# flucoma/flucoma-core

Hardware: AMD Instinct MI355X
Metric: NMF iterations/sec (buffer-iterations over the whole BufNMF job: STFT + 200-iter KL-NMF + write-back), rank-32 fft2048 (higher is better)
Workload: dtype f64; 1 GPU; BASELINE config 4 shard: 128 x 10 s mono 44.1 kHz buffers per GPU, fft 2048 / hop 512, rank 32, 200 iterations, seed 42; buffers_per_gpu=128, samples=441000, frames=862, bins=1025, rank=32, parallelism=single

## Files before the change

### flucoma-core_amd/csrc/kernels_nmf5.hip

```cpp
#include "fluhip_kernels.h"
#include "recip_tree.h"

#include <cstdlib>

namespace fluhip {

typedef double d2 __attribute__((ext_vector_type(2)));

struct Upd5Args
{
  const double* V;
  int64_t ldv, strideV;
  const double* Mv;
  int64_t strideM;
  double* S;
  int64_t strideS;
  int R, C, B;
  int nGroups, wavesPerBuf, wgPerBuf, nSteps, nsplit, stepsPerSplit;
  double* part;
  double* dpart;
  int64_t Cp;
  int xcdMap;
  const double* nrm;
  int nrmMode;
  double* statPart;
  long long* clk;
  const WaveDesc* list;
  double* sidePart;
  double* sideWold;
  const double* cmbStat;
  const double* cmbSide;
  const double* cmbWold;
  double* cmbNrmOut;
  double* cmbRowOut;
  int cmbParts, cmbSlices, cmbK;
  const double* colIn;
  double* colOut;
  int colInN;
};

#ifndef FLUHIP_QUOTIENT_CORRECTION
#define FLUHIP_QUOTIENT_CORRECTION 0
#endif
constexpr bool kQuotientCorrection = FLUHIP_QUOTIENT_CORRECTION != 0;
#ifndef FLUHIP_SHARED_RECIPROCAL
#define FLUHIP_SHARED_RECIPROCAL 1
#endif
constexpr bool kSharedReciprocal = FLUHIP_SHARED_RECIPROCAL != 0;
#ifndef FLUHIP_RCP_GROUP
#define FLUHIP_RCP_GROUP 4
#endif
constexpr int kRcpGroup = FLUHIP_RCP_GROUP;
#ifndef FLUHIP_QV_M10
#define FLUHIP_QV_M10 1
#endif
static_assert(kRcpGroup == 2 || kRcpGroup == 4 || kRcpGroup == 8, "quotients per reciprocal");
#ifndef FLUHIP_EPILOGUE_SC1
#define FLUHIP_EPILOGUE_SC1 1
#endif
__device__ __forceinline__ void store_result16(double* p, double __attribute__((ext_vector_type(2))) t)
{
#if FLUHIP_EPILOGUE_SC1 == 2
  asm volatile("global_store_dwordx4 %0, %1, off sc1 nt\n\ts_nop 1" ::"v"(p), "v"(t) : "memory");
#elif FLUHIP_EPILOGUE_SC1 == 3
  asm volatile("global_store_dwordx4 %0, %1, off nt\n\ts_nop 1" ::"v"(p), "v"(t) : "memory");
#elif FLUHIP_EPILOGUE_SC1 == 4
  asm volatile("global_store_dwordx4 %0, %1, off sc0 sc1\n\ts_nop 1" ::"v"(p), "v"(t) : "memory");
#elif FLUHIP_EPILOGUE_SC1
  asm volatile("global_store_dwordx4 %0, %1, off sc1\n\ts_nop 1" ::"v"(p), "v"(t) : "memory");
#else
  *reinterpret_cast<double __attribute__((ext_vector_type(2)))*>(p) = t;
#endif
}

__device__ __forceinline__ double fdiv_pos(double v, double d)
{
  double y = __builtin_amdgcn_rcp(d);
  const double e = __builtin_fma(-d, y, 1.0);
  y = __builtin_fma(y, e, y);
  const double r = v * y;
  const double res = __builtin_fma(-d, r, v);
  return __builtin_fma(res, y, r);
}

#define FLUHIP_GLDS(src, dst)                                                                     \
  __builtin_amdgcn_global_load_lds((const __attribute__((address_space(1))) void*) (src),          \
                                   (__attribute__((address_space(3))) void*) (dst), 16, 0, 0)

__device__ __forceinline__ void glds16(const void* sbase, unsigned voff, unsigned ldsAddr)
{
  asm volatile("s_mov_b32 m0, %0\n\ts_nop 0\n\tglobal_load_lds_dwordx4 %1, %2"
               :
               : "s"(ldsAddr), "v"(voff), "s"(sbase)
               : "memory", "m0");
}
#ifndef FLUHIP_PARTIAL_STAGED
#define FLUHIP_PARTIAL_STAGED 1
#endif
#ifndef FLUHIP_V_NT
#define FLUHIP_V_NT 1
#endif
__device__ __forceinline__ void glds16_v(const void* sbase, unsigned voff, unsigned ldsAddr)
{
#if FLUHIP_V_NT
  asm volatile("s_mov_b32 m0, %0\n\ts_nop 0\n\tglobal_load_lds_dwordx4 %1, %2 nt"
               :
               : "s"(ldsAddr), "v"(voff), "s"(sbase)
               : "memory", "m0");
#else
  glds16(sbase, voff, ldsAddr);
#endif
}
__device__ __forceinline__ unsigned lds_addr(const void* p)
{
  return (unsigned) (size_t) (__attribute__((address_space(3))) const void*) p;
}

template <int N>
__device__ __forceinline__ void load_vec5(double (&dst)[N], const double* p)
{
#pragma unroll
  for (int j = 0; j < N; j += 2)
  {
    d2 t = *reinterpret_cast<const d2*>(p + j);
    dst[j] = t[0];
    dst[j + 1] = t[1];
  }
}
#ifndef FLUHIP_STATIONARY_NT
#define FLUHIP_STATIONARY_NT 0
#endif
template <int N>
__device__ __forceinline__ void load_stationary5(double (&dst)[N], const double* p)
{
#if FLUHIP_STATIONARY_NT
#pragma unroll
  for (int j = 0; j < N; j += 2)
  {
    d2 t = __builtin_nontemporal_load(reinterpret_cast<const d2*>(p + j));
    dst[j] = t[0];
    dst[j + 1] = t[1];
  }
#else
  load_vec5<N>(dst, p);
#endif
}

template <int CTRL>
__device__ __forceinline__ double quad_dpp(double v)
{
  const long long b = __double_as_longlong(v);
  const int lo = __builtin_amdgcn_update_dpp(0, (int) (b & 0xffffffff), CTRL, 0xf, 0xf, false);
  const int hi = __builtin_amdgcn_update_dpp(0, (int) (b >> 32), CTRL, 0xf, 0xf, false);
  return __longlong_as_double(((long long) hi << 32) | (unsigned) lo);
}

template <int M, int NG, int NS, int WPS, int INSTR = 0, int MODE = 0, int DS = 1, int LIST = 0, int SIDEQ = 0, int KPM = 4 * M>
__global__ __launch_bounds__(256 * WPS, WPS) void nmf_update5_kernel(Upd5Args a)
{
  constexpr int KP = 4 * M;
  static_assert(KPM >= KP && KPM % 16 == 0, "array rank");
  constexpr int SPR = KP / 2;
  constexpr int NJV = (32 * NG + 63) / 64;
  constexpr int NJM = (4 * SPR + 63) / 64;
  constexpr int VSTAGE = NJV * 1024;
  constexpr int MSTAGE = NJM * 1024;
  constexpr int WAVE_LDS = NS * (VSTAGE + MSTAGE);
  constexpr int IPS = NJV + NJM;
  constexpr bool QV = MODE == 1 && (DS == 2 || (DS == 1 && INSTR == 0 && (M == 4 || (M == 6 && NG <= 8) || (M == 8 && NG <= 6) || (FLUHIP_QV_M10 && M == 10 && NG <= 4))));
  constexpr int STG_BYTES = (NG * M + M) * 512;
  constexpr int WAVE_REGION = (LIST != 0 && STG_BYTES > WAVE_LDS && 4 * STG_BYTES <= 160 * 1024) ? STG_BYTES : WAVE_LDS;

  extern __shared__ __attribute__((aligned(16))) char lds[];

  int id = blockIdx.x;
  int buf, wg, split;
  [[maybe_unused]] const WaveDesc* wd = nullptr;
  if constexpr (LIST != 0)
  {
    wd = a.list + ((int64_t) id * 4 * WPS + __builtin_amdgcn_readfirstlane(threadIdx.x >> 6));
    buf = __builtin_amdgcn_readfirstlane(wd->buf);
    wg = 0; split = 0;
  }
  else
  {
  if (a.xcdMap)
  {
    const int xcd = id & 7;
    int slot = id >> 3;
    split = slot % a.nsplit;
    slot /= a.nsplit;
    wg = slot % a.wgPerBuf;
    buf = xcd + 8 * (slot / a.wgPerBuf);
  }
  else
  {
    split = id % a.nsplit;
    wg = (id / a.nsplit) % a.wgPerBuf;
    buf = id / (a.nsplit * a.wgPerBuf);
  }
  if (buf >= a.B) return;
  }
  long long tEntry = 0;
  if constexpr (INSTR) tEntry = (long long) __builtin_amdgcn_s_memrealtime();
  long long clkC0 = 0, clkR0 = 0;
  const bool stamp = a.clk != nullptr && blockIdx.x == 0;
  if (stamp)
  {
    clkC0 = (long long) __builtin_readcyclecounter();
    clkR0 = (long long) __builtin_amdgcn_s_memrealtime();
  }
  const int lane = threadIdx.x & 63;
  const int wave = __builtin_amdgcn_readfirstlane(threadIdx.x >> 6);
  constexpr int WPB = 4 * WPS;
  const int strip = wg * WPB + wave;
  int g0 = 0, ng = 0;
  if constexpr (LIST != 0)
  {
    g0 = __builtin_amdgcn_readfirstlane(wd->g0);
    ng = __builtin_amdgcn_readfirstlane(wd->ng);
  }
  else
  {
  if (strip >= a.wavesPerBuf) return;
  const int base = a.nGroups / a.wavesPerBuf, rem = a.nGroups % a.wavesPerBuf;
  {
    const int nPairs = (a.wavesPerBuf + WPS - 1) / WPS;
    int acc0 = 0;
    for (int st = 0; st <= strip; st++)
    {
      const int wgi = st / WPB, w = st % WPB;
      const int pair = wgi * 4 + (w & 3), member = w >> 2;
      const int extra = (pair + nPairs * member) < rem ? 1 : 0;
      const int cnt = base + extra;
      if (st == strip) { g0 = acc0; ng = cnt; }
      acc0 += cnt;
    }
  }
  }
  if (ng <= 0) return;

  const int x = lane & 3, blk = (lane >> 2) & 3, y = lane >> 4;
  const double* __restrict__ V = a.V + (int64_t) buf * a.strideV;
  const double* __restrict__ Mv = a.Mv + (int64_t) buf * a.strideM;
  double* S = a.S + (int64_t) buf * a.strideS;

  char* vring = lds + wave * WAVE_REGION;
  char* mring = vring + NS * VSTAGE;

  unsigned voffs[NJV];
#pragma unroll
  for (int j = 0; j < NJV; j++)
  {
    int i = 64 * j + lane;
    int row = i / (8 * NG), cc = i % (8 * NG);
    if (row > 3) { row = 3; }
    cc = min(cc, 8 * ng - 1);
    voffs[j] = (unsigned) ((row * a.ldv + cc * 2) * 8);
  }
  unsigned moffs[NJM];
#pragma unroll
  for (int j = 0; j < NJM; j++)
  {
    int p = 64 * j + lane;
    int row = p / SPR, pos = p % SPR;
    if (row > 3) row = 3;
    const int cs = (pos - row + SPR) % SPR;
    const int cx = cs ^ (((cs >> 4) & 3) << 2);
    const int c = cx < SPR ? cx : cs;
    moffs[j] = (unsigned) ((row * KPM + c * 2) * 8);
  }

  int s0, s1;
  if constexpr (LIST != 0)
  {
    s0 = __builtin_amdgcn_readfirstlane(wd->s0);
    s1 = __builtin_amdgcn_readfirstlane(wd->s1);
  }
  else
  {
    s0 = split * a.stepsPerSplit;
    s1 = min(s0 + a.stepsPerSplit, a.nSteps);
  }
  const int sLast = s1 - 1;

  auto issue_stage = [&](int st) {
    const int sc = min(st, sLast);
    const int slot = st % NS;
    const char* vsrc = reinterpret_cast<const char*>(V + (int64_t) sc * 4 * a.ldv + (int64_t) g0 * 16);
    const char* msrc = reinterpret_cast<const char*>(Mv + (int64_t) sc * 4 * KPM);
#pragma unroll
    for (int j = 0; j < NJV; j++) FLUHIP_GLDS(vsrc + voffs[j], vring + slot * VSTAGE + j * 1024);
#pragma unroll
    for (int j = 0; j < NJM; j++) FLUHIP_GLDS(msrc + moffs[j], mring + slot * MSTAGE + j * 1024);
  };

  auto fill_slots = [&](int t0, int t1) {
    if (s0 < s1)
    {
#pragma unroll
      for (int t = t0; t < t1; t++)
      {
        const int sc = min(s0 + t, sLast);
        const char* vsrc = reinterpret_cast<const char*>(V + (int64_t) sc * 4 * a.ldv + (int64_t) g0 * 16);
        const char* msrc = reinterpret_cast<const char*>(Mv + (int64_t) sc * 4 * KPM);
#pragma unroll
        for (int j = 0; j < NJV; j++) FLUHIP_GLDS(vsrc + voffs[j], vring + t * VSTAGE + j * 1024);
#pragma unroll
        for (int j = 0; j < NJM; j++) FLUHIP_GLDS(msrc + moffs[j], mring + t * MSTAGE + j * 1024);
      }
    }
  };
  long long tP1 = 0, tP2 = 0, tP3 = 0;
  if constexpr (INSTR) tP1 = (long long) __builtin_amdgcn_s_memrealtime();
  constexpr int NJSV = SIDEQ ? (NG * 128 + 1023) / 1024 : 0;
  constexpr bool NORMQ = (SIDEQ & 2) != 0;
  [[maybe_unused]] char* sideL = nullptr;
  [[maybe_unused]] double cs[8], cm[8], cn[8], cd[8], cwo = 0.0, cc[8];
  static_assert(DS != 2 || NORMQ || SIDEQ == 0, "DS == 2: the W update's plain form or the H update's norm form");
  if constexpr (DS == 2)
  {
#pragma unroll
    for (int u = 0; u < 8; u++) cc[u] = 0.0;
    if (lane < KP)
    {
      const int64_t rec = NORMQ ? KPM : 2 * KPM;
      const double* cp = a.colIn + (int64_t) buf * a.colInN * rec + (NORMQ ? 0 : KPM) + lane;
#pragma unroll
      for (int u = 0; u < 8; u++) if (u < a.colInN) cc[u] = cp[(int64_t) u * rec];
    }
  }
  if constexpr (NORMQ)
  {
#pragma unroll
    for (int u = 0; u < 8; u++) { cs[u] = 0.0; cm[u] = -INFINITY; cn[u] = 0.0; cd[u] = 0.0; }
    if (lane < KP)
    {
      const double* sp = a.cmbStat + (int64_t) buf * a.cmbParts * 2 * KPM + lane;
      const double* qp = a.cmbSide + (int64_t) buf * a.cmbSlices * 2 * KPM + lane;
      cwo = a.cmbWold[(int64_t) buf * KPM + lane];
#pragma unroll
      for (int u = 0; u < 8; u++)
      {
        if (u < a.cmbParts) { cs[u] = sp[(int64_t) u * 2 * KPM]; cm[u] = sp[(int64_t) u * 2 * KPM + KPM]; }
        if (u < a.cmbSlices) { cn[u] = qp[(int64_t) u * 2 * KPM]; cd[u] = qp[(int64_t) u * 2 * KPM + KPM]; }
      }
    }
  }
  constexpr int SIDE_BYTES = SIDEQ ? (1 + NJSV) * 1024 : 0;
  constexpr int EXTRA_BYTES = SIDE_BYTES + (DS == 2 ? 512 : 0);
  [[maybe_unused]] double* colL = reinterpret_cast<double*>(lds + WPB * WAVE_REGION + wave * EXTRA_BYTES + SIDE_BYTES);
  if constexpr (SIDEQ)
  {
    sideL = lds + WPB * WAVE_REGION + wave * EXTRA_BYTES;
    if constexpr (!NORMQ)
    {
      const char* wsrc = reinterpret_cast<const char*>(Mv + (int64_t) (a.R - 1) * KPM) + min(lane, SPR - 1) * 16;
      FLUHIP_GLDS(wsrc, sideL);
    }
#pragma unroll
    for (int j = 0; j < NJSV; j++)
    {
      const int i = min(64 * j + lane, 8 * ng - 1);
      const char* vsrc = reinterpret_cast<const char*>(V + (int64_t) (a.R - 1) * a.ldv + (int64_t) g0 * 16) + i * 16;
      FLUHIP_GLDS(vsrc, sideL + 1024 + j * 1024);
    }
  }
  if constexpr (MODE >= 1) fill_slots(0, 2);

  double sb[NG][M];
  double acc[NG][M];
#pragma unroll
  for (int g = 0; g < NG; g++)
  {
#pragma unroll
    for (int m = 0; m < M; m++) { acc[g][m] = 0.0; sb[g][m] = 0.0; }
    if (g < ng) load_stationary5<M>(sb[g], S + (int64_t) ((g0 + g) * 16 + 4 * blk + x) * KPM + M * y);
  }
  [[maybe_unused]] double colSum = 0.0;
  if constexpr (DS == 2)
  {
#pragma unroll
    for (int u = 0; u < 8; u++) colSum += cc[u];
    if (lane < KP)
    {
      const int64_t rec = NORMQ ? KPM : 2 * KPM;
      const double* cp = a.colIn + (int64_t) buf * a.colInN * rec + (NORMQ ? 0 : KPM) + lane;
      for (int j = 8; j < a.colInN; j++) colSum += cp[(int64_t) j * rec];
    }
    if constexpr (!NORMQ)
    {
      if (lane < KP) colL[lane] = colSum;
      asm volatile("s_waitcnt lgkmcnt(0)" ::: "memory");
    }
  }
  if constexpr (NORMQ)
  {
    double t = 0.0, mv = -INFINITY, n = 0.0, d = 0.0;
#pragma unroll
    for (int u = 0; u < 8; u++) { t += cs[u]; mv = fmax(mv, cm[u]); n += cn[u]; d += cd[u]; }
    if (lane < KP)
    {
      const double* sp = a.cmbStat + (int64_t) buf * a.cmbParts * 2 * KPM + lane;
      const double* qp = a.cmbSide + (int64_t) buf * a.cmbSlices * 2 * KPM + lane;
      for (int j = 8; j < a.cmbParts; j++) { t += sp[(int64_t) j * 2 * KPM]; mv = fmax(mv, sp[(int64_t) j * 2 * KPM + KPM]); }
      for (int j = 8; j < a.cmbSlices; j++) { n += qp[(int64_t) j * 2 * KPM]; d += qp[(int64_t) j * 2 * KPM + KPM]; }
    }
    const bool liveK = lane < a.cmbK;
    const double wnew = liveK ? (cwo * n) / fmax(d, kEpsilon) : 0.0;
    t = __builtin_fma(wnew, wnew, t);
    mv = liveK ? fmax(mv, wnew) : -INFINITY;
#pragma unroll
    for (int off = 1; off < 64; off <<= 1) mv = fmax(mv, __shfl_xor(mv, off));
    const double nv = (liveK && mv > kEpsilon) ? sqrt(t) : 1.0;
    double* ldsW = reinterpret_cast<double*>(sideL);
    if (lane < KP)
    {
      ldsW[lane] = wnew;
      ldsW[64 + lane] = nv;
      if constexpr (DS == 2) colL[lane] = colSum + wnew;
      a.cmbRowOut[(int64_t) buf * a.strideM + (int64_t) (a.R - 1) * KPM + lane] = wnew;
      if (strip == 0) a.cmbNrmOut[(int64_t) buf * KPM + lane] = nv;
    }
    asm volatile("s_waitcnt lgkmcnt(0)" ::: "memory");
  }
  if (a.nrmMode)
  {
    double nr[M];
    if constexpr (NORMQ)
    {
      const double* ldsN = reinterpret_cast<const double*>(sideL) + 64;
#pragma unroll
      for (int m = 0; m < M; m++) nr[m] = ldsN[M * y + m];
    }
    else
    load_vec5<M>(nr, a.nrm + (int64_t) buf * KPM + M * y);
#pragma unroll
    for (int g = 0; g < NG; g++)
#pragma unroll
      for (int m = 0; m < M; m++) sb[g][m] = fdiv_pos(sb[g][m], nr[m]);
  }
  if constexpr (INSTR)
  {
    __builtin_amdgcn_sched_barrier(0);
    asm volatile("" ::"v"(sb[0][0]), "v"(sb[NG - 1][M - 1]));
    tP2 = (long long) __builtin_amdgcn_s_memrealtime();
    __builtin_amdgcn_sched_barrier(0);
  }
  if constexpr (MODE >= 1) fill_slots(2, NS);
  double dsum[M];
#pragma unroll
  for (int m = 0; m < M; m++) dsum[m] = 0.0;

  auto slot_of = [](int c, int r) { const int cx = c ^ (((c >> 4) & 3) << 2); return ((cx < SPR ? cx : c) + r) % SPR; };
  int maOff[M / 2], mbOff[M / 2];
#pragma unroll
  for (int j = 0; j < M / 2; j++)
  {
    maOff[j] = x * (KP * 8) + slot_of((M / 2) * y + j, x) * 16;
    mbOff[j] = y * (KP * 8) + slot_of((M / 2) * x + j, y) * 16;
  }
  const int vOff = y * (NG * 128) + (4 * blk + x) * 8;

  auto read_ma = [&](int st, double (&ma)[M]) {
    const char* mp = mring + (st % NS) * MSTAGE;
#pragma unroll
    for (int j = 0; j < M / 2; j++)
    {
      d2 t = *reinterpret_cast<const d2*>(mp + maOff[j]);
      ma[2 * j] = t[0];
      ma[2 * j + 1] = t[1];
    }
  };
  auto read_v = [&](int st, double (&v)[NG]) {
    const char* vp = vring + (st % NS) * VSTAGE + vOff;
#pragma unroll
    for (int g = 0; g < NG; g++) v[g] = *reinterpret_cast<const double*>(vp + g * 128);
  };
  auto read_mb = [&](int st, double (&mb)[M]) {
    const char* mp = mring + (st % NS) * MSTAGE;
#pragma unroll
    for (int j = 0; j < M / 2; j++)
    {
      d2 t = *reinterpret_cast<const d2*>(mp + mbOff[j]);
      mb[2 * j] = t[0];
      mb[2 * j + 1] = t[1];
    }
  };

  constexpr int P0 = (NG >= 5) ? 1 : (NG >= 3 ? 2 : (NG >= 2 ? 4 : 8));
  constexpr int P = (M % P0 == 0 || M < P0) ? P0 : (M == 12 ? P0 / 2 : P0);
  auto q_phase = [&](const double (&ma)[M], double (&q)[NG]) {
    constexpr int PP = (P <= M) ? P : M;
    double qp[NG][PP];
#pragma unroll
    for (int g = 0; g < NG; g++)
#pragma unroll
      for (int p = 0; p < PP; p++) qp[g][p] = 0.0;
#pragma unroll
    for (int m = 0; m < M; m++)
#pragma unroll
      for (int g = 0; g < NG; g++)
        qp[g][m % PP] = __builtin_amdgcn_mfma_f64_4x4x4f64(ma[m], sb[g][m], qp[g][m % PP], 0, 0, 0);
#pragma unroll
    for (int g = 0; g < NG; g++)
    {
      double t = qp[g][0];
#pragma unroll
      for (int p = 1; p < PP; p++) t += qp[g][p];
      q[g] = t;
    }
  };
  auto ratio_phase = [&](const double (&v)[NG], const double (&q)[NG], double (&ratio)[NG]) {
    double d[NG], yv[NG];
#pragma unroll
    for (int g = 0; g < NG; g++) d[g] = q[g] > kEpsilon ? q[g] : kEpsilon;
    if constexpr (kQuotientCorrection || !kSharedReciprocal)
    {
#pragma unroll
      for (int g = 0; g < NG; g++) yv[g] = __builtin_amdgcn_rcp(d[g]);
#pragma unroll
      for (int g = 0; g < NG; g++) ratio[g] = __builtin_fma(-d[g], yv[g], 1.0);
#pragma unroll
      for (int g = 0; g < NG; g++) yv[g] = __builtin_fma(yv[g], ratio[g], yv[g]);
    }
    else if constexpr (kRcpGroup > 2)
    {
      recip_tree<NG, kRcpGroup>(d, yv);
    }
    else
    {
      constexpr int NP = NG / 2;
      double pr[NP > 0 ? NP : 1], rr[NP > 0 ? NP : 1], ee[NP > 0 ? NP : 1];
#pragma unroll
      for (int h = 0; h < NP; h++) pr[h] = d[2 * h] * d[2 * h + 1];
#pragma unroll
      for (int h = 0; h < NP; h++) rr[h] = __builtin_amdgcn_rcp(pr[h]);
      if constexpr (NG & 1) yv[NG - 1] = __builtin_amdgcn_rcp(d[NG - 1]);
#pragma unroll
      for (int h = 0; h < NP; h++) ee[h] = __builtin_fma(-pr[h], rr[h], 1.0);
      if constexpr (NG & 1) ratio[NG - 1] = __builtin_fma(-d[NG - 1], yv[NG - 1], 1.0);
#pragma unroll
      for (int h = 0; h < NP; h++) rr[h] = __builtin_fma(rr[h], ee[h], rr[h]);
      if constexpr (NG & 1) yv[NG - 1] = __builtin_fma(yv[NG - 1], ratio[NG - 1], yv[NG - 1]);
#pragma unroll
      for (int h = 0; h < NP; h++)
      {
        yv[2 * h] = rr[h] * d[2 * h + 1];
        yv[2 * h + 1] = rr[h] * d[2 * h];
      }
    }
#pragma unroll
    for (int g = 0; g < NG; g++) ratio[g] = v[g] * yv[g];
    if constexpr (kQuotientCorrection)
    {
#pragma unroll
      for (int g = 0; g < NG; g++) d[g] = __builtin_fma(-d[g], ratio[g], v[g]);
#pragma unroll
      for (int g = 0; g < NG; g++) ratio[g] = __builtin_fma(d[g], yv[g], ratio[g]);
    }
  };
  auto out_phase = [&](const double (&ratio)[NG], const double (&mb)[M]) {
#pragma unroll
    for (int g = 0; g < NG; g++)
#pragma unroll
      for (int m = 0; m < M; m++) acc[g][m] = __builtin_amdgcn_mfma_f64_4x4x4f64(ratio[g], mb[m], acc[g][m], 0, 0, 0);
#pragma unroll
    for (int m = 0; m < M; m++) if constexpr (DS == 1) dsum[m] += mb[m];
  };

  if constexpr (MODE == 2)
  {
    if (s0 < s1)
    {
      static_assert(NS >= 4, "overlapped pipeline: ring depth >= 4");
      const unsigned vringA = __builtin_amdgcn_readfirstlane(lds_addr(vring));
      const unsigned mringA = __builtin_amdgcn_readfirstlane(lds_addr(mring));
      const char* vAddr = vring + vOff;
      const char* maAddr[M / 2];
      const char* mbAddr[M / 2];
#pragma unroll
      for (int j = 0; j < M / 2; j++) { maAddr[j] = mring + maOff[j]; mbAddr[j] = mring + mbOff[j]; }
      double v[NG], ma[M], mb[M], qA[NG], qB[NG];
      asm volatile("s_waitcnt vmcnt(%0)" ::"n"((NS - 2) * IPS) : "memory");
#pragma unroll
      for (int j = 0; j < M / 2; j++)
      {
        d2 t = *reinterpret_cast<const d2*>(maAddr[j]);
        ma[2 * j] = t[0]; ma[2 * j + 1] = t[1];
      }
      q_phase(ma, qA);
#pragma unroll
      for (int g = 0; g < NG; g++) v[g] = *reinterpret_cast<const double*>(vAddr + g * 128);
#pragma unroll
      for (int j = 0; j < M / 2; j++)
      {
        d2 t = *reinterpret_cast<const d2*>(mbAddr[j]);
        mb[2 * j] = t[0]; mb[2 * j + 1] = t[1];
        d2 t2 = *reinterpret_cast<const d2*>(maAddr[j] + MSTAGE);
        ma[2 * j] = t2[0]; ma[2 * j + 1] = t2[1];
      }
      constexpr int NMF = M * NG;
// ... 252 lines not shown
#pragma unroll
            for (int p = 1; p < PP; p++) t += qp[g][p];
            qn[g] = t;
          }
        }
        const long long c4 = tick();
        if constexpr (INSTR) { tWait += c1 - c0; tRatio += c2 - c1; tQ += c3 - c2; tOut += c4 - c3; }
      };
      for (int s = s0; s < s1; s += NS)
      {
#pragma unroll
        for (int u = 0; u < NS; u++)
        {
          if (s + u >= s1) break;
          if (u % 2 == 0) half(s + u, u, (u + 1) % NS, (u + 2) % NS, vX, maX, mbX, vY, maY, mbY, qA, qB);
          else half(s + u, u, (u + 1) % NS, (u + 2) % NS, vY, maY, mbY, vX, maX, mbX, qB, qA);
        }
      }
      asm volatile("s_waitcnt vmcnt(0)" ::: "memory");
      if constexpr (INSTR)
      {
        const long long tLoop1 = (long long) __builtin_amdgcn_s_memrealtime();
        tReal += tLoop1;
        if (blockIdx.x == 17 && threadIdx.x == 0 && a.dpart)
        {
          long long* o = reinterpret_cast<long long*>(a.dpart);
          o[0] = tWait; o[1] = 0; o[2] = tRatio; o[3] = tQ; o[4] = tOut; o[5] = 0; o[6] = s1 - s0; o[7] = tReal;
        }
        if (threadIdx.x == 0 && a.dpart && (blockIdx.x & 63) == 17)
        {
          long long* o = reinterpret_cast<long long*>(a.dpart) + 16 + 4 * (blockIdx.x >> 6);
          o[0] = tEntry; o[1] = tLoop0; o[2] = tLoop1;
          if (blockIdx.x == 17) { long long* q = reinterpret_cast<long long*>(a.dpart) + 12; q[0] = tP1; q[1] = tP2; q[2] = tP3; }
        }
      }
    }
  }
  else
  if (s0 < s1)
  {
#pragma unroll
    for (int t = 0; t < NS; t++) issue_stage(s0 + t);
    double ma[M], mb[M], v[NG], qA[NG], qB[NG], ratio[NG];
    asm volatile("s_waitcnt vmcnt(%0)" ::"n"((NS - 1) * IPS) : "memory");
    read_ma(s0, ma);
    q_phase(ma, qA);
    long long tWait = 0, tRead = 0, tRatio = 0, tQ = 0, tOut = 0, tDma = 0;
    auto tick = [&]() -> long long {
      if constexpr (INSTR) { __builtin_amdgcn_sched_barrier(0); long long c = __builtin_readcyclecounter(); __builtin_amdgcn_sched_barrier(0); return c; }
      return 0;
    };
    for (int s = s0; s < s1; s += 2)
    {
      long long c0 = tick();
      asm volatile("s_waitcnt vmcnt(%0)" ::"n"((NS - 2) * IPS) : "memory");
      long long c1 = tick();
      read_v(s, v);
      read_ma(s + 1, ma);
      read_mb(s, mb);
      asm volatile("s_waitcnt lgkmcnt(0)" ::: "memory");
      long long c2 = tick();
      issue_stage(s + NS);
      long long c3 = tick();
      ratio_phase(v, qA, ratio);
      long long c4 = tick();
      q_phase(ma, qB);
      long long c5 = tick();
      out_phase(ratio, mb);
      long long c6 = tick();
      if constexpr (INSTR) { tWait += c1 - c0; tRead += c2 - c1; tDma += c3 - c2; tRatio += c4 - c3; tQ += c5 - c4; tOut += c6 - c5; }
      if (s + 1 < s1)
      {
        asm volatile("s_waitcnt vmcnt(%0)" ::"n"((NS - 2) * IPS) : "memory");
        read_v(s + 1, v);
        read_ma(s + 2, ma);
        read_mb(s + 1, mb);
        asm volatile("s_waitcnt lgkmcnt(0)" ::: "memory");
        issue_stage(s + 1 + NS);
        ratio_phase(v, qB, ratio);
        q_phase(ma, qA);
        out_phase(ratio, mb);
      }
    }
    asm volatile("s_waitcnt vmcnt(0)" ::: "memory");
    if constexpr (INSTR)
    {
      if (blockIdx.x == 17 && threadIdx.x == 0 && a.dpart)
      {
        long long* o = reinterpret_cast<long long*>(a.dpart);
        o[0] = tWait; o[1] = tRead; o[2] = tRatio; o[3] = tQ; o[4] = tOut; o[5] = tDma; o[6] = (s1 - s0 + 1) / 2;
      }
    }
  }

  [[maybe_unused]] int lPart = -1, lStat = 0, lD = -1;
  if constexpr (LIST != 0 && 4 * STG_BYTES <= 160 * 1024)
  {
    const int grp = __builtin_amdgcn_readfirstlane(wd->grp);
    if (grp >> 16)
    {
      const int leader = grp & 15, rank = (grp >> 4) & 15, gsize = (grp >> 8) & 15;
      double* mine = reinterpret_cast<double*>(lds + wave * WAVE_REGION);
      if (rank > 0)
      {
#pragma unroll
        for (int g = 0; g < NG; g++)
#pragma unroll
          for (int m = 0; m < M; m++) mine[(g * M + m) * 64 + lane] = acc[g][m];
#pragma unroll
        for (int m = 0; m < M; m++) mine[(NG * M + m) * 64 + lane] = dsum[m];
      }
      __syncthreads();
      if (rank > 0) return;
      for (int r = 1; r < gsize; r++)
      {
        const double* src = reinterpret_cast<const double*>(lds + (leader + r) * WAVE_REGION);
#pragma unroll
        for (int g = 0; g < NG; g++)
#pragma unroll
          for (int m = 0; m < M; m++) acc[g][m] += src[(g * M + m) * 64 + lane];
#pragma unroll
        for (int m = 0; m < M; m++) dsum[m] += src[(NG * M + m) * 64 + lane];
      }
    }
  }
  if constexpr (LIST != 0)
  {
    lPart = __builtin_amdgcn_readfirstlane(wd->partIdx);
    lStat = __builtin_amdgcn_readfirstlane(wd->statIdx);
    lD = __builtin_amdgcn_readfirstlane(wd->dIdx);
  }
  auto whole = [&]() -> bool { if constexpr (LIST != 0) return lPart < 0; else return a.nsplit == 1; };
  if constexpr (DS == 1)
  {
#pragma unroll
    for (int m = 0; m < M; m++)
    {
      double d = dsum[m];
      d += __shfl_xor(d, 16);
      d += __shfl_xor(d, 32);
      dsum[m] = d;
    }
  }
  else if constexpr (DS == 2)
  {
#pragma unroll
    for (int m = 0; m < M; m++) dsum[m] = colL[M * x + m];
  }
  else if (whole())
  {
    load_vec5<M>(dsum, a.dpart + (int64_t) buf * KPM + M * x);
  }

  if (whole())
  {
    double nrE[M], ss[M], mx[M];
    [[maybe_unused]] double csum[M];
    constexpr bool COLOUT = DS == 2 && !NORMQ;
    [[maybe_unused]] double nrL = 1.0;
    if constexpr (NORMQ)
    {
      const double* ldsN = reinterpret_cast<const double*>(sideL) + 64;
#pragma unroll
      for (int m = 0; m < M; m++) nrE[m] = ldsN[M * x + m];
      if (lane < KP) nrL = ldsN[lane];
    }
    else
    {
      if (a.nrmMode) load_vec5<M>(nrE, a.nrm + (int64_t) buf * KPM + M * x);
      if constexpr (SIDEQ) if (strip == 0 && lane < KP) nrL = a.nrm[(int64_t) buf * KPM + lane];
    }
    if (a.nrmMode == 2)
    {
#pragma unroll
      for (int m = 0; m < M; m++) dsum[m] = fdiv_pos(dsum[m], nrE[m]);
    }
    double dd[M], dy[M];
#pragma unroll
    for (int m = 0; m < M; m++)
    {
      dd[m] = fmax(dsum[m], kEpsilon);
      double y0 = __builtin_amdgcn_rcp(dd[m]);
      dy[m] = __builtin_fma(y0, __builtin_fma(-dd[m], y0, 1.0), y0);
      ss[m] = 0.0;
      mx[m] = -INFINITY;
      if constexpr (COLOUT) csum[m] = 0.0;
    }
    const int srcLane = y + 4 * blk + 16 * x;
    constexpr int ROWB = KP * 8 + 16;
    constexpr int GRPB = 16 * ROWB;
    constexpr int GB = (WAVE_LDS / GRPB) >= NG ? NG : (WAVE_LDS / GRPB);
    static_assert(GB >= 1, "result staging does not fit the ring");
    constexpr int CPR = KP / 2;
    constexpr int NST = 16 * CPR / 64;
    char* stg = lds + wave * WAVE_REGION;
    [[maybe_unused]] double wsd[M], numS[M], denS[M], vsd[NG];
    if constexpr (SIDEQ)
    {
      static_assert(KP <= 64 && LIST == 0, "side-column partials: one lane per component at the end");
      const double* wl = reinterpret_cast<const double*>(sideL);
      const double* vl = reinterpret_cast<const double*>(sideL + 1024);
#pragma unroll
      for (int m = 0; m < M; m++) { wsd[m] = fdiv_pos(wl[M * x + m], nrE[m]); numS[m] = 0.0; denS[m] = 0.0; }
#pragma unroll
      for (int g = 0; g < NG; g++)
      {
        const int col = (g0 + g) * 16 + 4 * blk + y;
        vsd[g] = (g < ng && col < a.C) ? vl[g * 16 + 4 * blk + y] : 0.0;
      }
    }
#pragma unroll
    for (int gb = 0; gb < NG; gb += GB)
    {
#pragma unroll
      for (int g = gb; g < gb + GB && g < NG; g++)
      {
        const int col = (g0 + g) * 16 + 4 * blk + y;
        const bool live = g < ng && col < a.C;
        char* row = stg + (g - gb) * GRPB + (4 * blk + y) * ROWB + (M * x) * 8;
        [[maybe_unused]] double rr[M];
#pragma unroll
        for (int m = 0; m < M; m += 2)
        {
          double r2[2];
#pragma unroll
          for (int e = 0; e < 2; e++)
          {
            const double so = __shfl(sb[g][m + e], srcLane);
            const double v = so * acc[g][m + e];
            const double r0 = v * dy[m + e];
            const double r = __builtin_fma(__builtin_fma(-dd[m + e], r0, v), dy[m + e], r0);
            r2[e] = r;
            if constexpr (SIDEQ) rr[m + e] = r;
            if (live)
            {
              ss[m + e] = __builtin_fma(r, r, ss[m + e]);
              mx[m + e] = fmax(mx[m + e], r);
              if constexpr (COLOUT) csum[m + e] += r;
            }
          }
          *reinterpret_cast<d2*>(row + m * 8) = d2{r2[0], r2[1]};
        }
        if constexpr (SIDEQ)
        {
          double qs = 0.0;
#pragma unroll
          for (int m = 0; m < M; m++) qs = __builtin_fma(rr[m], wsd[m], qs);
          qs += quad_dpp<0xB1>(qs);
          qs += quad_dpp<0x4E>(qs);
          const double ratio = live ? fdiv_pos(vsd[g], fmax(qs, kEpsilon)) : 0.0;
#pragma unroll
          for (int m = 0; m < M; m++)
          {
            numS[m] = __builtin_fma(ratio, rr[m], numS[m]);
            denS[m] += live ? rr[m] : 0.0;
          }
        }
      }
#pragma unroll
      for (int g = gb; g < gb + GB && g < NG; g++)
      {
        if (g < ng)
        {
#pragma unroll
          for (int j = 0; j < NST; j++)
          {
            const int c = 64 * j + lane;
            const int r = c / CPR, piece = c % CPR;
            const d2 t = *reinterpret_cast<const d2*>(stg + (g - gb) * GRPB + r * ROWB + piece * 16);
            const int col = (g0 + g) * 16 + r;
            if (col < a.C) store_result16(S + (int64_t) col * KPM + piece * 2, t);
          }
        }
      }
    }
    if constexpr (SIDEQ)
    {
      double* red = reinterpret_cast<double*>(stg);
      asm volatile("s_waitcnt lgkmcnt(0)" ::: "memory");
      const int jr = 4 * blk + y;
#pragma unroll
      for (int m = 0; m < M; m++)
      {
        red[jr * KP + M * x + m] = numS[m];
        red[(16 + jr) * KP + M * x + m] = denS[m];
      }
      asm volatile("s_waitcnt lgkmcnt(0)" ::: "memory");
      if (lane < KP)
      {
        double pn[16], pd[16];
#pragma unroll
        for (int j = 0; j < 16; j++) { pn[j] = red[j * KP + lane]; pd[j] = red[(16 + j) * KP + lane]; }
        double n = 0.0, d = 0.0;
#pragma unroll
        for (int j = 0; j < 16; j++) { n += pn[j]; d += pd[j]; }
        double* sp = a.sidePart + ((int64_t) buf * a.wavesPerBuf + strip) * 2 * KPM;
        sp[lane] = n;
        sp[KPM + lane] = d;
        if (strip == 0) a.sideWold[(int64_t) buf * KPM + lane] = reinterpret_cast<const double*>(sideL)[lane] / nrL;
      }
    }
    if (a.statPart)
    {
#pragma unroll
      for (int m = 0; m < M; m++)
      {
        double t = ss[m], u = mx[m];
#pragma unroll
        for (int off = 4; off < 64; off <<= 1)
        {
          t += __shfl_xor(t, off);
          u = fmax(u, __shfl_xor(u, off));
        }
        ss[m] = t;
        mx[m] = u;
      }
      if (lane < 4)
      {
        double* sp = a.statPart + (LIST ? (int64_t) lStat : ((int64_t) buf * a.wavesPerBuf + strip)) * 2 * KPM + M * x;
#pragma unroll
        for (int m = 0; m < M; m++) { sp[m] = ss[m]; sp[KPM + m] = mx[m]; }
      }
    }
    if constexpr (COLOUT)
    {
#pragma unroll
      for (int m = 0; m < M; m++)
      {
        double t = csum[m];
#pragma unroll
        for (int off = 4; off < 64; off <<= 1) t += __shfl_xor(t, off);
        csum[m] = t;
      }
      if (lane < 4)
      {
        double* cp = a.colOut + ((int64_t) buf * a.wavesPerBuf + strip) * KPM + M * x;
#pragma unroll
        for (int m = 0; m < M; m++) cp[m] = csum[m];
      }
    }
  }
  else
  {
    double* part = a.part + (LIST ? (int64_t) lPart : ((int64_t) buf * a.nsplit + split)) * a.Cp * KPM;
#if FLUHIP_PARTIAL_STAGED
    {
      constexpr int ROWB = KP * 8 + 16;
      constexpr int GRPB = 16 * ROWB;
      constexpr int GB = (WAVE_LDS / GRPB) >= NG ? NG : (WAVE_LDS / GRPB);
      static_assert(GB >= 1, "partial staging does not fit the ring");
      constexpr int CPR = KP / 2, NST = 16 * CPR / 64;
      char* stg = lds + wave * WAVE_REGION;
#pragma unroll
      for (int gb = 0; gb < NG; gb += GB)
      {
#pragma unroll
        for (int g = gb; g < gb + GB && g < NG; g++)
        {
          char* row = stg + (g - gb) * GRPB + (4 * blk + y) * ROWB + (M * x) * 8;
#pragma unroll
          for (int m = 0; m < M; m += 2) *reinterpret_cast<d2*>(row + m * 8) = d2{acc[g][m], acc[g][m + 1]};
        }
#pragma unroll
        for (int g = gb; g < gb + GB && g < NG; g++)
        {
          if (g < ng)
          {
#pragma unroll
            for (int j = 0; j < NST; j++)
            {
              const int c = 64 * j + lane;
              const int r = c / CPR, piece = c % CPR;
              const d2 t = *reinterpret_cast<const d2*>(stg + (g - gb) * GRPB + r * ROWB + piece * 16);
              store_result16(part + (int64_t) ((g0 + g) * 16 + r) * KPM + piece * 2, t);
            }
          }
        }
      }
    }
#else
#pragma unroll
    for (int g = 0; g < NG; g++)
    {
      if (g < ng)
      {
        const int col = (g0 + g) * 16 + 4 * blk + y;
        double* pp = part + (int64_t) col * KPM + M * x;
#pragma unroll
        for (int m = 0; m < M; m++) pp[m] = acc[g][m];
      }
    }
#endif
    if (DS && (LIST ? lD >= 0 : strip == 0) && blk == 0 && y == 0)
    {
      double* dp = a.dpart + (LIST ? (int64_t) lD : ((int64_t) buf * a.nsplit + split)) * KPM + M * x;
#pragma unroll
      for (int m = 0; m < M; m++) dp[m] = dsum[m];
    }
  }
  if (stamp && threadIdx.x == 0)
  {
    __builtin_amdgcn_s_waitcnt(0);
    const long long c1 = (long long) __builtin_readcyclecounter(), r1 = (long long) __builtin_amdgcn_s_memrealtime();
    a.clk[0] += 1;
    a.clk[1] += c1 - clkC0;
    a.clk[2] += r1 - clkR0;
  }
  if constexpr (INSTR)
  {
    __builtin_amdgcn_s_waitcnt(0);
    if (threadIdx.x == 0 && a.dpart && (blockIdx.x & 63) == 17)
      reinterpret_cast<long long*>(a.dpart)[16 + 4 * (blockIdx.x >> 6) + 3] = (long long) __builtin_amdgcn_s_memrealtime();
  }
}


template <int M, int NG, int NS, int MODE, int KPM = 4 * M>
static void launch5_list(const UpdateArgs& a, hipStream_t s)
{
  Upd5Args k{};
  k.V = a.V; k.ldv = a.ldv; k.strideV = a.strideV;
  k.Mv = a.Mv; k.strideM = a.strideM;
  k.S = a.S; k.strideS = a.strideS;
  k.R = a.R; k.C = a.C; k.B = a.B;
  k.nGroups = (a.C + 15) / 16;
  k.wavesPerBuf = 1; k.wgPerBuf = 1; k.nSteps = (a.R + 3) / 4; k.nsplit = 1; k.stepsPerSplit = k.nSteps;
  k.part = a.part; k.dpart = a.dpart; k.Cp = a.Cp;
  k.nrm = a.nrm; k.nrmMode = a.nrmMode; k.statPart = a.listPartial ? nullptr : a.statPart;
  k.clk = a.clk; k.xcdMap = 0; k.list = a.list;
  constexpr int KP = 4 * M, SPR = KP / 2;
  constexpr int NJV = (32 * NG + 63) / 64, NJM = (4 * SPR + 63) / 64;
  constexpr size_t ring = (size_t) NS * (NJV + NJM) * 1024, stg = (size_t) (NG * M + M) * 512;
  constexpr size_t shmem = 4 * ((stg > ring && 4 * stg <= 160 * 1024) ? stg : ring);
  static_assert(shmem <= 160 * 1024, "LDS");
  auto kern = nmf_update5_kernel<M, NG, NS, 1, 0, MODE, 1, 1, 0, KPM>;
  request_dynamic_lds(kern, (size_t) (shmem));
  hipLaunchKernelGGL(kern, dim3((unsigned) a.listWGs), dim3(256), shmem, s, k);
}

template <int M, int NG, int NS, int WPS, int INSTR = 0, int MODE = 0, int DS = 1, int SIDEQ = 0, int KPM = 4 * M>
static void launch5_t(const UpdateArgs& a, int wavesPerBuf, hipStream_t s)
{
  Upd5Args k;
  if (a.dryRun) return;
  k.sidePart = SIDEQ ? a.sideOut : nullptr; k.sideWold = SIDEQ ? a.sideWold : nullptr;
  k.cmbStat = a.cmbStat; k.cmbSide = a.cmbSide; k.cmbWold = a.cmbWold; k.cmbNrmOut = a.cmbNrmOut; k.cmbRowOut = a.cmbRowOut;
  k.cmbParts = a.cmbParts; k.cmbSlices = a.cmbSlices; k.cmbK = a.cmbK;
  k.colIn = a.colIn; k.colOut = a.colOut; k.colInN = a.colInN;
  k.V = a.V; k.ldv = a.ldv; k.strideV = a.strideV;
  k.Mv = a.Mv; k.strideM = a.strideM;
  k.S = a.S; k.strideS = a.strideS;
  k.R = a.R; k.C = a.C; k.B = a.B;
  k.nGroups = (a.C + 15) / 16;
  k.wavesPerBuf = wavesPerBuf;
  k.wgPerBuf = (wavesPerBuf + 4 * WPS - 1) / (4 * WPS);
  k.nSteps = (a.R + 3) / 4;
  k.nsplit = a.nsplit < 1 ? 1 : a.nsplit;
  k.stepsPerSplit = (k.nSteps + k.nsplit - 1) / k.nsplit;
  k.part = a.part; k.dpart = a.dpart; k.Cp = a.Cp;
  k.nrm = a.nrm; k.nrmMode = a.nrmMode; k.statPart = a.nsplit > 1 ? nullptr : a.statPart;
  k.clk = a.clk;
  k.xcdMap = a.B >= 8 ? 1 : 0;
  k.list = nullptr;
  const int bufs = k.xcdMap ? (int) round_up(a.B, 8) : a.B;
  const unsigned grid = (unsigned) (bufs * k.wgPerBuf * k.nsplit);
  constexpr int KP = 4 * M, SPR = KP / 2;
  constexpr int NJV = (32 * NG + 63) / 64, NJM = (4 * SPR + 63) / 64;
  constexpr size_t shmem = (size_t) 4 * WPS * ((NS * (NJV + NJM) + (SIDEQ ? 1 + (NG * 128 + 1023) / 1024 : 0)) * 1024 + (DS == 2 ? 512 : 0));
  static_assert(shmem <= 160 * 1024, "LDS ring does not fit");
  auto kern = nmf_update5_kernel<M, NG, NS, WPS, INSTR, MODE, DS, 0, SIDEQ, KPM>;
  request_dynamic_lds(kern, (size_t) (shmem));
  hipLaunchKernelGGL(kern, dim3(grid), dim3(256 * WPS), shmem, s, k);
  if (k.nsplit > 1)
    launch_update_finalize(a.S, a.strideS, a.part, a.dpart, a.C, a.Kp, a.Cp, k.nsplit, a.B, s, a.nrm, a.nrmMode,
                           a.statPart);
}

#ifndef FLUHIP_K5_OFFSIZE_TU
static int max_groups(int M)
{
  if (M <= 8) return 9;
  if (M <= 16) return 4;
  return 2;
}

int nmf_update5_waves_per_buffer(int C, int Kp, int B)
{
  const int M = Kp / 4, G = (C + 15) / 16, ngmax = max_groups(M);
  const int wmin = (G + ngmax - 1) / ngmax;
  static const int forceW = [] { const char* e = fluhip::ab_getenv("FLUHIP_PLAN_W"); return e ? std::atoi(e) : 0; }();
  if (forceW > 0) return forceW < wmin ? wmin : (forceW > G ? G : forceW);
  int w = wmin;
  const int simds = 1024;
  if ((int64_t) B * w >= simds)
  {
    for (int cand = wmin; cand <= wmin + 2 && cand <= G; cand++)
      if (((int64_t) B * cand) % simds == 0) { w = cand; break; }
  }
  else
  {
    const int64_t wfill = (simds + B - 1) / B;
    if (wfill <= G / 3 || wfill <= wmin)
      w = (int) std::max<int64_t>(wmin, wfill);
    else
      w = std::max(wmin, (G + 2) / 3);
    if (w > G) w = G;
    if (w < 1) w = 1;
  }
  return w;
}


#endif

template <int M, int NG, int WPS>
constexpr int ring_depth()
{
  constexpr int NJ = (32 * NG + 63) / 64 + (4 * (2 * M) + 63) / 64;
  constexpr int fit = 160 / (4 * WPS * NJ);
  return fit >= 6 ? 6 : (fit < 3 ? 3 : fit);
}

#ifndef FLUHIP_K5_OFFSIZE_TU
template <int M, int NG, int WPS>
static int launch5_ng(const UpdateArgs& a, int w, int ng, hipStream_t s)
{
  if constexpr (NG == 1) launch5_t<M, 1, ring_depth<M, 1, WPS>(), WPS>(a, w, s);
  else
  {
    const bool sideq = a.sideOut && a.sideWold && a.nrmMode == 2 && a.nsplit <= 1 && w <= kSideFromHSlots;
// ... 254 lines not shown
```

Baseline: 244,900 iterations/s.

## Software-pipeline epilogue staging with double-buffered LDS areas and scalar-base immediate-offset stores

Restructures the update kernel's epilogue so each 16-column group's results are staged into one of two LDS areas while the previous group is read back and stored to global memory, replacing the batch-then-store loop. Global stores now use an SGPR base plus a 32-bit lane offset and compile-time immediate offsets, which cuts 64-bit address arithmetic per store. The side-quotient math can be deferred behind the stores, and shuffle batching is tuned by M. An optional flag (off by default) moves the ring prefill earlier. Risks are higher register pressure and changed LDS reuse hazards when only one staging area fits.

```diff
diff --git a/flucoma-core_amd/csrc/kernels_nmf5.hip b/flucoma-core_amd/csrc/kernels_nmf5.hip
--- a/flucoma-core_amd/csrc/kernels_nmf5.hip
+++ b/flucoma-core_amd/csrc/kernels_nmf5.hip
@@ -2,6 +2,7 @@
 #include "recip_tree.h"
 
 #include <cstdlib>
+#include <type_traits>
 
 namespace fluhip {
 
@@ -58,19 +59,33 @@
 #ifndef FLUHIP_EPILOGUE_SC1
 #define FLUHIP_EPILOGUE_SC1 1
 #endif
-__device__ __forceinline__ void store_result16(double* p, double __attribute__((ext_vector_type(2))) t)
-{
 #if FLUHIP_EPILOGUE_SC1 == 2
-  asm volatile("global_store_dwordx4 %0, %1, off sc1 nt\n\ts_nop 1" ::"v"(p), "v"(t) : "memory");
+#define FLUHIP_STORE_POLICY " sc1 nt"
 #elif FLUHIP_EPILOGUE_SC1 == 3
-  asm volatile("global_store_dwordx4 %0, %1, off nt\n\ts_nop 1" ::"v"(p), "v"(t) : "memory");
+#define FLUHIP_STORE_POLICY " nt"
 #elif FLUHIP_EPILOGUE_SC1 == 4
-  asm volatile("global_store_dwordx4 %0, %1, off sc0 sc1\n\ts_nop 1" ::"v"(p), "v"(t) : "memory");
-#elif FLUHIP_EPILOGUE_SC1
-  asm volatile("global_store_dwordx4 %0, %1, off sc1\n\ts_nop 1" ::"v"(p), "v"(t) : "memory");
+#define FLUHIP_STORE_POLICY " sc0 sc1"
 #else
-  *reinterpret_cast<double __attribute__((ext_vector_type(2)))*>(p) = t;
-#endif
+#define FLUHIP_STORE_POLICY " sc1"
+#endif
+template <int IMM>
+__device__ __forceinline__ void store_result16(const char* sbase, unsigned voff, double __attribute__((ext_vector_type(2))) t)
+{
+  static_assert(IMM >= 0 && IMM < 4096, "immediate offset of a global store");
+#if FLUHIP_EPILOGUE_SC1
+  asm volatile("global_store_dwordx4 %0, %1, %2 offset:%3" FLUHIP_STORE_POLICY "\n\ts_nop 1" ::"v"(voff), "v"(t), "s"(sbase), "n"(IMM) : "memory");
+#else
+  *reinterpret_cast<double __attribute__((ext_vector_type(2)))*>(const_cast<char*>(sbase) + voff + IMM) = t;
+#endif
+}
+template <int J, int N, class F>
+__device__ __forceinline__ void static_for5(F&& f)
+{
+  if constexpr (J < N)
+  {
+    f(std::integral_constant<int, J>{});
+    static_for5<J + 1, N>(f);
+  }
 }
 
 __device__ __forceinline__ double fdiv_pos(double v, double d)
@@ -129,6 +144,9 @@
 }
 #ifndef FLUHIP_STATIONARY_NT
 #define FLUHIP_STATIONARY_NT 0
+#endif
+#ifndef FLUHIP_EARLY_RING
+#define FLUHIP_EARLY_RING 0
 #endif
 template <int N>
 __device__ __forceinline__ void load_stationary5(double (&dst)[N], const double* p)
@@ -377,6 +395,12 @@
     for (int m = 0; m < M; m++) { acc[g][m] = 0.0; sb[g][m] = 0.0; }
     if (g < ng) load_stationary5<M>(sb[g], S + (int64_t) ((g0 + g) * 16 + 4 * blk + x) * KPM + M * y);
   }
+  [[maybe_unused]] double nrFirst[M];
+  if constexpr (MODE >= 1 && FLUHIP_EARLY_RING)
+  {
+    if constexpr (!NORMQ) if (a.nrmMode) load_vec5<M>(nrFirst, a.nrm + (int64_t) buf * KPM + M * y);
+    fill_slots(2, NS);
+  }
   [[maybe_unused]] double colSum = 0.0;
   if constexpr (DS == 2)
   {
@@ -433,6 +457,11 @@
 #pragma unroll
       for (int m = 0; m < M; m++) nr[m] = ldsN[M * y + m];
     }
+    else if constexpr (MODE >= 1 && FLUHIP_EARLY_RING)
+    {
+#pragma unroll
+      for (int m = 0; m < M; m++) nr[m] = nrFirst[m];
+    }
     else
     load_vec5<M>(nr, a.nrm + (int64_t) buf * KPM + M * y);
 #pragma unroll
@@ -447,7 +476,7 @@
     tP2 = (long long) __builtin_amdgcn_s_memrealtime();
     __builtin_amdgcn_sched_barrier(0);
   }
-  if constexpr (MODE >= 1) fill_slots(2, NS);
+  if constexpr (MODE >= 1 && !FLUHIP_EARLY_RING) fill_slots(2, NS);
   double dsum[M];
 #pragma unroll
   for (int m = 0; m < M; m++) dsum[m] = 0.0;
@@ -1006,6 +1035,44 @@
     load_vec5<M>(dsum, a.dpart + (int64_t) buf * KPM + M * x);
   }
 
+  constexpr int ROWB = KP * 8 + 16;
+  constexpr int GRPB = 16 * ROWB;
+  static_assert(WAVE_LDS >= GRPB, "result staging does not fit the ring");
+  constexpr int NAREA = WAVE_LDS >= 2 * GRPB ? 2 : 1;
+  constexpr int CPR = KP / 2;
+  constexpr int NST = 16 * CPR / 64;
+  constexpr int NSB = M <= 8 ? NST : (M <= 14 ? 4 : 1);
+  char* const stg = lds + wave * WAVE_REGION;
+  auto read_pieces = [&](const char* area, auto jb, d2 (&t)[NSB]) __attribute__((always_inline)) {
+    constexpr int j0 = decltype(jb)::value * NSB, jn = (NST - j0) < NSB ? (NST - j0) : NSB;
+#pragma unroll
+    for (int j = 0; j < jn; j++)
+    {
+      const int c = 64 * (j0 + j) + lane, r = c / CPR, piece = c % CPR;
+      t[j] = *reinterpret_cast<const d2*>(area + r * ROWB + piece * 16);
+    }
+  };
+  auto store_pieces = [&](const double* dst, int rowsLive, auto jb, const d2 (&t)[NSB]) __attribute__((always_inline)) {
+    constexpr int j0 = decltype(jb)::value * NSB, jn = (NST - j0) < NSB ? (NST - j0) : NSB;
+    const char* db = reinterpret_cast<const char*>(dst);
+    auto put = [&](auto jc, bool guard) __attribute__((always_inline)) {
+      constexpr int j = j0 + decltype(jc)::value;
+      const int c = 64 * j + lane, r = c / CPR, piece = c % CPR;
+      if (guard && r >= rowsLive) return;
+      if constexpr (KPM == KP) store_result16<(j & 3) * 1024>(db + (j >> 2) * 4096, (unsigned) lane * 16u, t[j - j0]);
+      else store_result16<0>(db, (unsigned) ((r * KPM + piece * 2) * 8), t[j - j0]);
+    };
+    if (rowsLive >= 16) static_for5<0, jn>([&](auto jc) { put(jc, false); });
+    else static_for5<0, jn>([&](auto jc) { put(jc, true); });
+  };
+  auto store_group = [&](const char* area, const double* dst, int rowsLive) __attribute__((always_inline)) {
+    static_for5<0, (NST + NSB - 1) / NSB>([&](auto jb) {
+      d2 t[NSB];
+      read_pieces(area, jb, t);
+      store_pieces(dst, rowsLive, jb, t);
+    });
+  };
+
   if (whole())
   {
     double nrE[M], ss[M], mx[M];
@@ -1041,13 +1108,6 @@
       if constexpr (COLOUT) csum[m] = 0.0;
     }
     const int srcLane = y + 4 * blk + 16 * x;
-    constexpr int ROWB = KP * 8 + 16;
-    constexpr int GRPB = 16 * ROWB;
-    constexpr int GB = (WAVE_LDS / GRPB) >= NG ? NG : (WAVE_LDS / GRPB);
-    static_assert(GB >= 1, "result staging does not fit the ring");
-    constexpr int CPR = KP / 2;
-    constexpr int NST = 16 * CPR / 64;
-    char* stg = lds + wave * WAVE_REGION;
     [[maybe_unused]] double wsd[M], numS[M], denS[M], vsd[NG];
     if constexpr (SIDEQ)
     {
@@ -1063,69 +1123,69 @@
         vsd[g] = (g < ng && col < a.C) ? vl[g * 16 + 4 * blk + y] : 0.0;
       }
     }
-#pragma unroll
-    for (int gb = 0; gb < NG; gb += GB)
-    {
-#pragma unroll
-      for (int g = gb; g < gb + GB && g < NG; g++)
-      {
-        const int col = (g0 + g) * 16 + 4 * blk + y;
-        const bool live = g < ng && col < a.C;
-        char* row = stg + (g - gb) * GRPB + (4 * blk + y) * ROWB + (M * x) * 8;
-        [[maybe_unused]] double rr[M];
-#pragma unroll
-        for (int m = 0; m < M; m += 2)
+    [[maybe_unused]] double rr[M];
+    constexpr int SHB = M <= 8 ? M : 2;
+    constexpr bool SIDE_LATE = M <= 14;
+    auto side_math = [&](int g) __attribute__((always_inline)) {
+      const int col = (g0 + g) * 16 + 4 * blk + y;
+      const bool live = col < a.C;
+      double qs = 0.0;
+#pragma unroll
+      for (int m = 0; m < M; m++) qs = __builtin_fma(rr[m], wsd[m], qs);
+      qs += quad_dpp<0xB1>(qs);
+      qs += quad_dpp<0x4E>(qs);
+      const double ratio = live ? fdiv_pos(vsd[g], fmax(qs, kEpsilon)) : 0.0;
+#pragma unroll
+      for (int m = 0; m < M; m++)
+      {
+        numS[m] = __builtin_fma(ratio, rr[m], numS[m]);
+        denS[m] += live ? rr[m] : 0.0;
+      }
+    };
+    auto group_math = [&](int g) __attribute__((always_inline)) {
+      const int col = (g0 + g) * 16 + 4 * blk + y;
+      const bool live = col < a.C;
+      char* row = stg + (g % NAREA) * GRPB + (4 * blk + y) * ROWB + (M * x) * 8;
+      double so[SHB];
+#pragma unroll
+      for (int m = 0; m < M; m += 2)
+      {
+        if (m % SHB == 0)
         {
-          double r2[2];
-#pragma unroll
-          for (int e = 0; e < 2; e++)
+#pragma unroll
+          for (int u = 0; u < SHB; u++) so[u] = __shfl(sb[g][m + u], srcLane);
+        }
+        double r2[2];
+#pragma unroll
+        for (int e = 0; e < 2; e++)
+        {
+          const double v = so[(m + e) % SHB] * acc[g][m + e];
+          const double r0 = v * dy[m + e];
+          const double r = __builtin_fma(__builtin_fma(-dd[m + e], r0, v), dy[m + e], r0);
+          r2[e] = r;
+          if constexpr (SIDEQ) rr[m + e] = r;
+          if (live)
           {
-            const double so = __shfl(sb[g][m + e], srcLane);
-            const double v = so * acc[g][m + e];
-            const double r0 = v * dy[m + e];
-            const double r = __builtin_fma(__builtin_fma(-dd[m + e], r0, v), dy[m + e], r0);
-            r2[e] = r;
-            if constexpr (SIDEQ) rr[m + e] = r;
-            if (live)
-            {
-              ss[m + e] = __builtin_fma(r, r, ss[m + e]);
-              mx[m + e] = fmax(mx[m + e], r);
-              if constexpr (COLOUT) csum[m + e] += r;
-            }
-          }
-          *reinterpret_cast<d2*>(row + m * 8) = d2{r2[0], r2[1]};
-        }
-        if constexpr (SIDEQ)
-        {
-          double qs = 0.0;
-#pragma unroll
-          for (int m = 0; m < M; m++) qs = __builtin_fma(rr[m], wsd[m], qs);
-          qs += quad_dpp<0xB1>(qs);
-          qs += quad_dpp<0x4E>(qs);
-          const double ratio = live ? fdiv_pos(vsd[g], fmax(qs, kEpsilon)) : 0.0;
-#pragma unroll
-          for (int m = 0; m < M; m++)
-          {
-            numS[m] = __builtin_fma(ratio, rr[m], numS[m]);
-            denS[m] += live ? rr[m] : 0.0;
+            ss[m + e] = __builtin_fma(r, r, ss[m + e]);
+            mx[m + e] = fmax(mx[m + e], r);
+            if constexpr (COLOUT) csum[m + e] += r;
           }
         }
-      }
-#pragma unroll
-      for (int g = gb; g < gb + GB && g < NG; g++)
-      {
-        if (g < ng)
-        {
-#pragma unroll
-          for (int j = 0; j < NST; j++)
-          {
-            const int c = 64 * j + lane;
-            const int r = c / CPR, piece = c % CPR;
-            const d2 t = *reinterpret_cast<const d2*>(stg + (g - gb) * GRPB + r * ROWB + piece * 16);
-            const int col = (g0 + g) * 16 + r;
-            if (col < a.C) store_result16(S + (int64_t) col * KPM + piece * 2, t);
-          }
-        }
+        *reinterpret_cast<d2*>(row + m * 8) = d2{r2[0], r2[1]};
+      }
+    };
+#pragma unroll
+    for (int g = 0; g <= NG; g++)
+    {
+      if (g > 0 && g - 1 < ng)
+      {
+        store_group(stg + ((g - 1) % NAREA) * GRPB, S + (int64_t) (g0 + g - 1) * 16 * KPM, a.C - (g0 + g - 1) * 16);
+        if constexpr (SIDEQ && SIDE_LATE) side_math(g - 1);
+      }
+      if (g < NG && g < ng)
+      {
+        group_math(g);
+        if constexpr (SIDEQ && !SIDE_LATE) side_math(g);
       }
     }
     if constexpr (SIDEQ)
@@ -1198,38 +1258,15 @@
   {
     double* part = a.part + (LIST ? (int64_t) lPart : ((int64_t) buf * a.nsplit + split)) * a.Cp * KPM;
 #if FLUHIP_PARTIAL_STAGED
-    {
-      constexpr int ROWB = KP * 8 + 16;
-      constexpr int GRPB = 16 * ROWB;
-      constexpr int GB = (WAVE_LDS / GRPB) >= NG ? NG : (WAVE_LDS / GRPB);
-      static_assert(GB >= 1, "partial staging does not fit the ring");
-      constexpr int CPR = KP / 2, NST = 16 * CPR / 64;
-      char* stg = lds + wave * WAVE_REGION;
-#pragma unroll
-      for (int gb = 0; gb < NG; gb += GB)
-      {
-#pragma unroll
-        for (int g = gb; g < gb + GB && g < NG; g++)
-        {
-          char* row = stg + (g - gb) * GRPB + (4 * blk + y) * ROWB + (M * x) * 8;
-#pragma unroll
-          for (int m = 0; m < M; m += 2) *reinterpret_cast<d2*>(row + m * 8) = d2{acc[g][m], acc[g][m + 1]};
-        }
-#pragma unroll
-        for (int g = gb; g < gb + GB && g < NG; g++)
-        {
-          if (g < ng)
-          {
-#pragma unroll
-            for (int j = 0; j < NST; j++)
-            {
-              const int c = 64 * j + lane;
-              const int r = c / CPR, piece = c % CPR;
-              const d2 t = *reinterpret_cast<const d2*>(stg + (g - gb) * GRPB + r * ROWB + piece * 16);
-              store_result16(part + (int64_t) ((g0 + g) * 16 + r) * KPM + piece * 2, t);
-            }
-          }
-        }
+#pragma unroll
+    for (int g = 0; g <= NG; g++)
+    {
+      if (g > 0 && g - 1 < ng) store_group(stg + ((g - 1) % NAREA) * GRPB, part + (int64_t) (g0 + g - 1) * 16 * KPM, 16);
+      if (g < NG && g < ng)
+      {
+        char* row = stg + (g % NAREA) * GRPB + (4 * blk + y) * ROWB + (M * x) * 8;
+#pragma unroll
+        for (int m = 0; m < M; m += 2) *reinterpret_cast<d2*>(row + m * 8) = d2{acc[g][m], acc[g][m + 1]};
       }
     }
 #else
```

Result: no change. 245,400 iterations/s (median of 6 runs) (+0.2%).
